# cjpurackal/nice-slam-cpp

Measured on AMD Instinct MI355X. Metric: mapping rays/sec (and ms/iter) on CoFusion room1 at 1/2/4/8 MI355X, higher is better.
Workload: dtype f32

## Files before the change

nice-slam-cpp_amd/csrc/nsk_train.h:

```cpp
#pragma once
#include "nsk_device.h"
#include <type_traits>
#include <utility>

#define PN_RB 272
#define PN_GROWS 32
#define PN_EROWS(CQ) (PN_GROWS + 16 * (CQ))
#define PN_ROWS(CQ) (PN_EROWS(CQ) + 96)
#define PN_MOFF(CQ) (PN_ROWS(CQ) * PN_RB)
#define PN_FLOATS(CQ) (2 * PN_MOFF(CQ) / 4)

struct TrainPhase {
    int RT, NC, rowsum;
    int slot0, nslots;
    int w_base, ld, col0;
    int rows, cols_total;
    int b_base;
};

template <int WHICH>
struct TrainPlan {
    static constexpr bool XYZ = WHICH != 0;
    static constexpr int CQ = WHICH == 2 ? 4 : 2;
    static constexpr int OD = WHICH == 3 ? 4 : 1;
// ... 191 lines not shown
                    else if (16 * ch + x < P.cols_total) g_dec[P.w_base + o * P.ld + P.col0 + 16 * ch + x] = v;
                }
            }
        }
    }
}

__device__ __forceinline__ void lds_barrier() { asm volatile("s_waitcnt lgkmcnt(0)\n\ts_barrier" ::: "memory"); }

template <int WHICH, bool RAYS, bool FULL = false>
__device__ __forceinline__ void decode_bwd_train_body(const DecArgs& A, int bid, int nb)
{
    constexpr bool XYZ = WHICH != 0;
    constexpr int CQ = WHICH == 2 ? 4 : 2;
    constexpr int OD = WHICH == 3 ? 4 : 1;
    constexpr bool SAVED = WHICH != 2;
    static_assert(FULL || WHICH == 0 || WHICH == 2, "the middle and colour decoders take this body only with FULL");
    typedef MlpFwdImg<CQ> FI;
    typedef TrainPlan<WHICH> PL;
    constexpr PL plan{};
    constexpr int BWD_F = XYZ ? MlpBwdImg::TOTAL : CoarseBwdImg::TOTAL;
    constexpr int IMG_F = SAVED ? BWD_F : 0;
    extern __shared__ __attribute__((aligned(16))) f4 smem[];
    const int wave = __builtin_amdgcn_readfirstlane(threadIdx.x >> 6), lane0 = threadIdx.x & 63;
    int lane = lane0, j = lane & 15, g = lane >> 4;
    float* smf = reinterpret_cast<float*>(smem);
    char* pn = reinterpret_cast<char*>(smf + IMG_F);
    constexpr int PM = PN_MOFF(CQ);
    float* scratch = smf + IMG_F + wave * 1056;
    copy_image_to_lds<512>(smem, A.bimg, IMG_F / 4);
    __syncthreads();
    const f4* fimg = A.img;
    const float* fimgf = reinterpret_cast<const float*>(fimg);
    const f4* bimg = SAVED ? smem : A.bimg;
    const float* bimgf = reinterpret_cast<const float*>(bimg);
    const float* Bm = nullptr;
    if constexpr (XYZ) Bm = SAVED ? bimgf + MlpBwdImg::P_BM : fimgf + FI::P_BM;
    const float* Bmb = Bm;
    const float* Wo = SAVED ? bimgf + (XYZ ? MlpBwdImg::P_WO : CoarseBwdImg::P_WO) : fimgf + FI::P_WO;

    f4 acc[plan.nslots];
#pragma unroll
    for (int k = 0; k < plan.nslots; ++k) acc[k] = (f4)(0.f);

    const int ntasks = (A.M + 15) >> 4;
    const int iters = tiles_per_wave(ntasks, nb * 8);
    const bool scat = (A.flags & 1u) && A.grid.g;
    struct Staged { float px, py, pz, zz; int n; bool valid; f4 gr; f4 xc[CQ]; f4 h4[2]; unsigned long long mask; } nx;
    auto task_of = [&](int it_) { return tile_of(it_, bid * 8 + wave, nb * 8); };
    auto slot_of = [&](int it_) { return task_of(it_) * 16 + j; };
    auto stage_a = [&](int it_, int mm, Staged& S_) {
        const int task = task_of(it_);
        const int slot = task * 16 + j;
        S_.valid = slot < A.M;
        sample_point(A, mm, S_.px, S_.py, S_.pz, S_.zz, S_.n);
        S_.gr = *reinterpret_cast<const f4*>(A.g_raw + (size_t)mm * 4);
        if constexpr (SAVED) {
            const int tk = min(task, ntasks - 1);
            S_.mask = A.masks[(size_t)min(slot, A.M - 1) * 4 + g];
            S_.h4[0] = A.hsave[((size_t)tk * 10 + 8) * 64 + lane]; S_.h4[1] = A.hsave[((size_t)tk * 10 + 9) * 64 + lane];
        }
    };
    auto stage_b = [&](Staged& S_) {
        Tri T_;
        tri_setup(A.grid, A.bound, S_.px, S_.py, S_.pz, T_);
        tri_gather(A.grid, T_, g, S_.xc[0], S_.xc[1]);
        if constexpr (WHICH == 2) {
            Tri Tm;
            tri_setup(A.grid_mid, A.bound, S_.px, S_.py, S_.pz, Tm);
            tri_gather(A.grid_mid, Tm, g, S_.xc[CQ - 2], S_.xc[CQ - 1]);
        }
    };
    int mm_next = 0;
    if (iters > 0) { stage_a(0, slot_sample(A, slot_of(0)), nx); stage_b(nx); mm_next = slot_sample(A, slot_of(1)); }
    if constexpr (SAVED) asm volatile("" : "+v"(nx.h4[0]), "+v"(nx.h4[1]), "+v"(nx.gr), "+v"(nx.mask), "+v"(mm_next));
    for (int it = 0; it < iters; ++it) {
        asm volatile("" ::: "memory");
        lane = lane0; asm volatile("" : "+v"(lane)); j = lane & 15; g = lane >> 4;
        if (it > 0) lds_barrier();
        const bool valid = nx.valid;
        float px = nx.px, py = nx.py, pz = nx.pz, zz = nx.zz; const int n = nx.n;
        Tri T;
        float gout[OD];
        {
            f4 gr = nx.gr;
            if (!valid) gr = (f4)(0.f);
            if constexpr (OD == 4) { gout[0] = gr[0]; gout[1] = gr[1]; gout[2] = gr[2]; gout[3] = 0.f; }
            else gout[0] = gr[3];
        }
        f4 go;
#pragma unroll
        for (int i = 0; i < 4; ++i) go[i] = (4 * g + i) < OD ? gout[(4 * g + i) < OD ? (4 * g + i) : 0] : 0.f;
        Act<CQ> C;
        ActC CC;
        f4 xcos[6];
        unsigned long long mask;
        const int htask = min(task_of(it), ntasks - 1);
        if constexpr (XYZ) {
#pragma unroll
            for (int q = 0; q < CQ; ++q) C.xc[q] = nx.xc[q];
            embed<false>(Bm, g, px, py, pz, C.xe, xcos);
#pragma unroll
            for (int q = 0; q < 6; ++q) pn_put(pn, PM, PN_EROWS(CQ) + 16 * q, wave, lane, C.xe[q]);
            if constexpr (SAVED) { C.h[4][0] = nx.h4[0]; C.h[4][1] = nx.h4[1]; mask = nx.mask; }
            else { mlp_forward<CQ>(fimg, lane, C); mask = C.mask; }
        } else {
            CC.xc[0] = nx.xc[0]; CC.xc[1] = nx.xc[1];
            CC.h[4][0] = nx.h4[0]; CC.h[4][1] = nx.h4[1]; mask = nx.mask;
        }
        f4 gh[2];
#pragma unroll
        for (int r = 0; r < 2; ++r)
#pragma unroll
            for (int i = 0; i < 4; ++i) {
                float s = 0.f;
#pragma unroll
                for (int o = 0; o < OD; ++o) s += Wo[32 * o + 16 * r + 4 * g + i] * gout[o];
                gh[r][i] = s;
            }
        {
            pn_put(pn, PM, 0, wave, lane, go);
            const f4* h4 = XYZ ? C.h[4] : CC.h[4];
            pn_put(pn, PM, PN_GROWS, wave, lane, h4[0]);
            pn_put(pn, PM, PN_GROWS + 16, wave, lane, h4[1]);
            lds_barrier();
            constexpr TrainPhase P = plan.p[PL::P_OUT];
            pn_tiles<P.nslots>(pn, PM, P.RT, P.NC, P.rowsum, wave, lane, acc + P.slot0);
            lds_barrier();
        }
        f4 gc[2] = {(f4)(0.f), (f4)(0.f)};
        f4 ge[6];
#pragma unroll
        for (int q = 0; q < 6; ++q) ge[q] = (f4)(0.f);
        auto load_h = [&](auto KC) {
            constexpr int k = decltype(KC)::value;
            const f4* src = A.hsave + ((size_t)htask * 10 + 2 * k) * 64 + lane;
            if constexpr (XYZ) { C.h[k][0] = src[0]; C.h[k][1] = src[64]; }
            else { CC.h[k][0] = src[0]; CC.h[k][1] = src[64]; }
        };
        if constexpr (SAVED) load_h(std::integral_constant<int, 3>{});
        auto layer = [&](auto LC) {
            constexpr int l = decltype(LC)::value;
            if constexpr (SAVED && l >= 2) load_h(std::integral_constant<int, l - 2>{});
            if constexpr (XYZ) {
                gemm<2, 2>(bimg, MlpBwdImg::FT(l), lane, gh, gc);
                pn_put(pn, PM, 0, wave, lane, gh[0]);
                pn_put(pn, PM, 16, wave, lane, gh[1]);
#pragma unroll
                for (int q = 0; q < CQ; ++q) pn_put(pn, PM, PN_GROWS + 16 * q, wave, lane, C.xc[q]);
                lds_barrier();
                constexpr TrainPhase P = plan.p[PL::P_FC0 + l];
                pn_tiles<P.nslots>(pn, PM, P.RT, P.NC, P.rowsum, wave, lane, acc + P.slot0);
                lds_barrier();
            }
            f4 ga[2];
#pragma unroll
            for (int r = 0; r < 2; ++r)
#pragma unroll
                for (int i = 0; i < 4; ++i) ga[r][i] = ((mask >> (8 * l + 4 * r + i)) & 1ull) ? gh[r][i] : 0.f;
            {
                pn_put(pn, PM, 0, wave, lane, ga[0]);
                pn_put(pn, PM, 16, wave, lane, ga[1]);
                if constexpr (XYZ) {
                    if constexpr (l == 0) {
                    } else if constexpr (l == 3) {
                        pn_put(pn, PM, PN_GROWS, wave, lane, C.h[2][0]);
                        pn_put(pn, PM, PN_GROWS + 16, wave, lane, C.h[2][1]);
                    } else {
                        pn_put(pn, PM, PN_GROWS, wave, lane, C.h[l - 1][0]);
                        pn_put(pn, PM, PN_GROWS + 16, wave, lane, C.h[l - 1][1]);
                    }
                } else {
                    if constexpr (l == 0 || l == 3) { pn_put(pn, PM, PN_GROWS, wave, lane, CC.xc[0]); pn_put(pn, PM, PN_GROWS + 16, wave, lane, CC.xc[1]); }
                    else { pn_put(pn, PM, PN_GROWS, wave, lane, CC.h[l - 1][0]); pn_put(pn, PM, PN_GROWS + 16, wave, lane, CC.h[l - 1][1]); }
                }
                lds_barrier();
                constexpr TrainPhase P = plan.p[PL::P_W0 + l];
                constexpr int xrow0 = (XYZ && (l == 0 || l == 3)) ? PN_EROWS(CQ) : PN_GROWS;
                pn_tiles<P.nslots>(pn, PM, P.RT, P.NC, P.rowsum, wave, lane, acc + P.slot0, xrow0);
                if constexpr (XYZ && l == 3) {
                    constexpr TrainPhase P2 = plan.p[PL::P_W3H];
                    pn_tiles<P2.nslots>(pn, PM, P2.RT, P2.NC, P2.rowsum, (wave + 4) & 7, lane, acc + P2.slot0);
                }
                lds_barrier();
                if constexpr (!XYZ && l == 3) {
                    const f4* h2 = CC.h[2];
                    pn_put(pn, PM, PN_GROWS, wave, lane, h2[0]);
                    pn_put(pn, PM, PN_GROWS + 16, wave, lane, h2[1]);
                    lds_barrier();
                    constexpr TrainPhase P2 = plan.p[PL::P_W3H];
                    pn_tiles<P2.nslots>(pn, PM, P2.RT, P2.NC, P2.rowsum, wave, lane, acc + P2.slot0);
                    lds_barrier();
                }
            }
            if constexpr (XYZ) {
                if constexpr (l == 3) gemm_e(bimg, MlpBwdImg::W3ET, lane, ga, ge);
                if constexpr (l == 0) gemm_e(bimg, MlpBwdImg::W0ET, lane, ga, ge);
                if constexpr (l >= 1) {
                    f4 ghn[2] = {(f4)(0.f), (f4)(0.f)};
                    gemm<2, 2>(bimg, MlpBwdImg::WT(l), lane, ga, ghn);
                    gh[0] = ghn[0]; gh[1] = ghn[1];
                }
            } else {
                if constexpr (l == 3) gemm<2, 2>(bimg, CoarseBwdImg::W3CT, lane, ga, gc);
                if constexpr (l == 0) gemm<2, 2>(bimg, CoarseBwdImg::W0T, lane, ga, gc);
                else {
                    constexpr int q0 = l == 1 ? CoarseBwdImg::W1T : (l == 2 ? CoarseBwdImg::W2T : (l == 3 ? CoarseBwdImg::W3HT : CoarseBwdImg::W4T));
                    f4 ghn[2] = {(f4)(0.f), (f4)(0.f)};
                    gemm<2, 2>(bimg, q0, lane, ga, ghn);
                    gh[0] = ghn[0]; gh[1] = ghn[1];
                }
            }
        };
        layer(std::integral_constant<int, 4>{});
        layer(std::integral_constant<int, 3>{});
        layer(std::integral_constant<int, 2>{});
        layer(std::integral_constant<int, 1>{});
        layer(std::integral_constant<int, 0>{});
        if (it + 1 < iters) { stage_a(it + 1, mm_next, nx); mm_next = slot_sample(A, slot_of(it + 2)); }
        float gp[3] = {0.f, 0.f, 0.f};
        asm volatile("" : "+v"(px), "+v"(py), "+v"(pz));
        tri_setup(A.grid, A.bound, px, py, pz, T);
        if constexpr (XYZ) {
            { f4 e2[6]; embed<true>(Bmb, g, px, py, pz, e2, xcos); }
#pragma unroll
            for (int q = 0; q < 6; ++q) ge[q] *= xcos[q];
            {
                f4 pq;
#pragma unroll
                for (int i = 0; i < 4; ++i) { int row = 4 * g + i; pq[i] = !valid ? 0.f : (row == 0 ? px : (row == 1 ? py : (row == 2 ? pz : 0.f))); }
                pn_put(pn, PM, 0, wave, lane, pq);
#pragma unroll
                for (int q = 0; q < 6; ++q) pn_put(pn, PM, PN_EROWS(CQ) + 16 * q, wave, lane, ge[q]);
                lds_barrier();
                constexpr TrainPhase P = plan.p[PL::P_DB];
                pn_tiles<P.nslots>(pn, PM, P.RT, P.NC, P.rowsum, wave, lane, acc + P.slot0, PN_EROWS(CQ));
                lds_barrier();
            }
            if constexpr (RAYS) {
#pragma unroll
                for (int q = 0; q < 6; ++q) {
                    f4 b0 = *reinterpret_cast<const f4*>(Bmb + 16 * q + 4 * g);
                    f4 b1 = *reinterpret_cast<const f4*>(Bmb + 96 + 16 * q + 4 * g);
                    f4 b2 = *reinterpret_cast<const f4*>(Bmb + 192 + 16 * q + 4 * g);
#pragma unroll
                    for (int i = 0; i < 4; ++i) { gp[0] += ge[q][i] * b0[i]; gp[1] += ge[q][i] * b1[i]; gp[2] += ge[q][i] * b2[i]; }
                }
            }
        }
        if constexpr (RAYS) {
            tri_grad_p(A.grid, T, g, gc, gp);
#pragma unroll
            for (int k = 0; k < 3; ++k) { gp[k] += __shfl_xor(gp[k], 16); gp[k] += __shfl_xor(gp[k], 32); }
            if (A.g_rays_o) {
                const int n0 = __builtin_amdgcn_readfirstlane(n);
                if (__builtin_amdgcn_ballot_w64(valid && n != n0) == 0ull) {
                    float a[6];
#pragma unroll
                    for (int k = 0; k < 3; ++k) { a[k] = valid ? gp[k] : 0.f; a[3 + k] = valid ? gp[k] * zz : 0.f; }
#pragma unroll
                    for (int o = 1; o < 16; o <<= 1)
#pragma unroll
                        for (int k = 0; k < 6; ++k) a[k] += __shfl_xor(a[k], o);
                    if (lane == 0) {
#pragma unroll
                        for (int k = 0; k < 3; ++k) { atomicAdd(A.g_rays_o + 3 * n0 + k, a[k]); atomicAdd(A.g_rays_d + 3 * n0 + k, a[3 + k]); }
                    }
                } else if (g == 0 && valid) {
#pragma unroll
                    for (int k = 0; k < 3; ++k) {
                        atomicAdd(A.g_rays_o + 3 * n + k, gp[k]);
                        atomicAdd(A.g_rays_d + 3 * n + k, gp[k] * zz);
                    }
                }
            }
        }
        if (it + 1 < iters) {
            stage_b(nx);
        }
        if constexpr (SAVED) asm volatile("" : "+v"(nx.h4[0]), "+v"(nx.h4[1]), "+v"(nx.gr), "+v"(nx.mask), "+v"(mm_next));
        if (scat) {
            if (A.flags & 0x8000u) {
                for (int w = 0; w < 8; ++w) { if (wave == w) { scatter_tile(A.grid, T, gc, lane, valid, scratch); asm volatile("s_waitcnt vmcnt(0)" ::: "memory"); } __syncthreads(); }
            } else scatter_tile(A.grid, T, gc, lane, valid, scratch);
        }
    }
    float* slab = A.g_dec + (size_t)bid * ((plan_total<WHICH>() + 3) & ~3);
    pn_flush<plan.p[PL::P_OUT].nslots>(slab, plan.p[PL::P_OUT], wave, lane, acc + plan.p[PL::P_OUT].slot0);
#define NSK_FLUSH(ID) if constexpr (plan.p[ID].nslots > 0) pn_flush<plan.p[ID].nslots>(slab, plan.p[ID], wave, lane, acc + plan.p[ID].slot0);
    NSK_FLUSH(1) NSK_FLUSH(2) NSK_FLUSH(3) NSK_FLUSH(4) NSK_FLUSH(5) NSK_FLUSH(6) NSK_FLUSH(7) NSK_FLUSH(8) NSK_FLUSH(9)
    NSK_FLUSH(10) NSK_FLUSH(12)
    if constexpr (plan.p[PL::P_W3H].nslots > 0)
        pn_flush<plan.p[PL::P_W3H].nslots>(slab, plan.p[PL::P_W3H], XYZ ? (wave + 4) & 7 : wave, lane, acc + plan.p[PL::P_W3H].slot0);
#undef NSK_FLUSH
}


#define PM_G1 0
#define PM_G2 32
#define PM_XC 64
#define PM_XH 96
#define PM_E 128
#define PM_ROWS 224
#define PM_IMG_FRAG_F (18 * 2 * 1024 / 4)
#define PM_IMG_F (PM_IMG_FRAG_F + 128 + 288)
#define PM_LDS_BYTES (PM_IMG_F * 4 + PM_ROWS * PN_RB * 2)

__device__ __forceinline__ void gemm_e2_lds(const h8* __restrict__ eimg, int lane, const H2& x3, const H2& x0, f4 (&acc)[6])
{
    constexpr int G3 = MlpBwdImgH::W3ET - MlpBwdImgH::W0ET;
#pragma unroll
    for (int a = 0; a < 3; ++a) {
        const FragH a30 = load_frag_h(eimg, G3 + 2 * a, lane), a31 = load_frag_h(eimg, G3 + 2 * a + 1, lane);
        const FragH a00 = load_frag_h(eimg, 2 * a, lane), a01 = load_frag_h(eimg, 2 * a + 1, lane);
        f4 tH[2] = {acc[2 * a], acc[2 * a + 1]}, tL[2] = {(f4)(0.f), (f4)(0.f)};
        mac_block_h(a30, a31, x3, tH, tL);
        mac_block_h(a00, a01, x0, tH, tL);
        acc[2 * a] = tH[0] + tL[0] * (1.f / NSK_H16_SCALE); acc[2 * a + 1] = tH[1] + tL[1] * (1.f / NSK_H16_SCALE);
    }
}
__device__ __forceinline__ void gemm_e2T_lds(const h8* __restrict__ eimg, int lane, const H2& x3, const H2& x0, f4 (&acc)[6])
{
    constexpr int G3 = MlpBwdImgH::W3ET - MlpBwdImgH::W0ET;
#pragma unroll
    for (int q = 0; q < 6; ++q) {
        const FragH f3 = load_frag_h(eimg, G3 + q, lane), f0 = load_frag_h(eimg, q, lane);
        f4 tH = (f4)(0.f), tL = (f4)(0.f);
        tH = mfma_h(x3.h, f3.h, tH); tL = mfma_h(x3.h, f3.l, tL); tL = mfma_h(x3.l, f3.h, tL);
        tH = mfma_h(x0.h, f0.h, tH); tL = mfma_h(x0.h, f0.l, tL); tL = mfma_h(x0.l, f0.h, tL);
        acc[q] = tH + tL * (1.f / NSK_H16_SCALE);
    }
}
typedef short s4v __attribute__((ext_vector_type(4)));
__device__ __forceinline__ f4 mfma_bf16_k16(unsigned a01, unsigned a23, unsigned b01, unsigned b23, f4 c)
{
    typedef unsigned int u2v __attribute__((ext_vector_type(2)));
    return __builtin_amdgcn_mfma_f32_16x16x16bf16_1k(__builtin_bit_cast(s4v, (u2v){a01, a23}), __builtin_bit_cast(s4v, (u2v){b01, b23}), c, 0, 0, 0);
}

struct TJob { int wave, grow, nt; int xrow[4]; int ph[4]; int rt; int ch[4]; };
template <int WHICH>
struct JobPlan {
    typedef TrainPlan<WHICH> PL;
    static constexpr int NJ = 32;
    static constexpr int PH_OUT = 0, PH_DB = 6;
    TJob j[NJ];
    int slot0[NJ];
    int first[8];
    int nslots;
    constexpr JobPlan() : j{}, slot0{}, first{}, nslots(0)
    {
        int n = 0;
        auto add = [&](int wave, int grow, int rt, int nt, int x0, int p0, int c0, int x1, int p1, int c1, int x2 = 0, int p2 = 0, int c2 = 0, int x3 = 0, int p3 = 0, int c3 = 0) {
            j[n] = TJob{wave, grow, nt, {x0, x1, x2, x3}, {p0, p1, p2, p3}, rt, {c0, c1, c2, c3}};
            ++n;
        };
        const int RS = -1;
        first[0] = n;
        add(0, PM_G1, 0, 3, PM_XH, PL::P_OUT, 0, PM_XH + 16, PL::P_OUT, 1, 0, PL::P_OUT, RS);
        for (int l = 4; l >= 0; --l) {
            first[1 + (4 - l)] = n;
            const int FC = PL::P_FC0 + l, W = PL::P_W0 + l;
            if (l == 4 || l == 2 || l == 1) {
                const int w0 = l == 4 ? 0 : 4;
                add(w0 + 0, PM_G1, 0, 3, PM_XC, FC, 0, PM_XC + 16, FC, 1, 0, FC, RS);
                add(w0 + 1, PM_G1 + 16, 1, 3, PM_XC, FC, 0, PM_XC + 16, FC, 1, 0, FC, RS);
                add(w0 + 2, PM_G2, 0, 3, PM_XH, W, 0, PM_XH + 16, W, 1, 0, W, RS);
                add(w0 + 3, PM_G2 + 16, 1, 3, PM_XH, W, 0, PM_XH + 16, W, 1, 0, W, RS);
            } else if (l == 3) {
                add(0, PM_G2, 0, 3, PM_E, W, 0, PM_E + 16, W, 1, 0, W, RS);
                add(4, PM_G1, 0, 3, PM_XC, FC, 0, PM_XC + 16, FC, 1, 0, FC, RS);
                add(1, PM_G2 + 16, 1, 3, PM_E, W, 0, PM_E + 16, W, 1, 0, W, RS);
                add(5, PM_G1 + 16, 1, 3, PM_XC, FC, 0, PM_XC + 16, FC, 1, 0, FC, RS);
                add(2, PM_G2, 0, 4, PM_E + 32, W, 2, PM_E + 48, W, 3, PM_XH, PL::P_W3H, 0, PM_XH + 16, PL::P_W3H, 1);
                add(6, PM_G2, 0, 2, PM_E + 64, W, 4, PM_E + 80, W, 5);
                add(3, PM_G2 + 16, 1, 4, PM_E + 32, W, 2, PM_E + 48, W, 3, PM_XH, PL::P_W3H, 0, PM_XH + 16, PL::P_W3H, 1);
                add(7, PM_G2 + 16, 1, 2, PM_E + 64, W, 4, PM_E + 80, W, 5);
            } else {
                add(0, PM_G2, 0, 3, PM_E, W, 0, PM_E + 16, W, 1, 0, W, RS);
                add(4, PM_G2, 0, 2, PM_E + 32, W, 2, PM_E + 48, W, 3);
                add(1, PM_G2 + 16, 1, 3, PM_E, W, 0, PM_E + 16, W, 1, 0, W, RS);
                add(5, PM_G2 + 16, 1, 2, PM_E + 32, W, 2, PM_E + 48, W, 3);
                add(2, PM_G1, 0, 3, PM_XC, FC, 0, PM_XC + 16, FC, 1, 0, FC, RS);
                add(6, PM_G2, 0, 2, PM_E + 64, W, 4, PM_E + 80, W, 5);
                add(3, PM_G1 + 16, 1, 3, PM_XC, FC, 0, PM_XC + 16, FC, 1, 0, FC, RS);
                add(7, PM_G2 + 16, 1, 2, PM_E + 64, W, 4, PM_E + 80, W, 5);
            }
        }
        first[6] = n;
        add(6, PM_G1, 0, 2, PM_E, PL::P_DB, 0, PM_E + 16, PL::P_DB, 1);
        add(7, PM_G1, 0, 2, PM_E + 32, PL::P_DB, 2, PM_E + 48, PL::P_DB, 3);
        add(1, PM_G1, 0, 2, PM_E + 64, PL::P_DB, 4, PM_E + 80, PL::P_DB, 5);
        first[7] = n;
        int used[8] = {0, 0, 0, 0, 0, 0, 0, 0};
        for (int q = 0; q < n; ++q) { slot0[q] = used[j[q].wave]; used[j[q].wave] += j[q].nt; }
        for (int w = 0; w < 8; ++w) nslots = used[w] > nslots ? used[w] : nslots;
    }
};

template <int WHICH>
constexpr bool jobplan_covers_plan()
{
    constexpr JobPlan<WHICH> JP{};
    constexpr TrainPlan<WHICH> plan{};
    for (int ph = 0; ph < TrainPlan<WHICH>::NPH; ++ph) {
        const TrainPhase P = plan.p[ph];
        for (int rt = 0; rt < P.RT; ++rt)
            for (int ch = -1; ch < P.NC; ++ch) {
                if (ch < 0 && !P.rowsum) continue;
                int owners = 0;
                for (int q = 0; q < JobPlan<WHICH>::NJ; ++q)
                    for (int k = 0; k < JP.j[q].nt; ++k)
                        if (JP.j[q].ph[k] == ph && JP.j[q].rt == rt && (ch < 0 ? JP.j[q].ch[k] < 0 : JP.j[q].ch[k] == ch)) ++owners;
                if (owners != 1) return false;
            }
    }
    int tiles = 0, want = 0;
    for (int q = 0; q < JobPlan<WHICH>::NJ; ++q) tiles += JP.j[q].nt;
    for (int ph = 0; ph < TrainPlan<WHICH>::NPH; ++ph) want += plan.p[ph].RT * plan.p[ph].NC + (plan.p[ph].rowsum ? plan.p[ph].RT : 0);
    return tiles == want && JP.nslots <= 12;
}
static_assert(jobplan_covers_plan<1>() && jobplan_covers_plan<3>(), "JobPlan: a weight-gradient tile is unowned, owned twice, or a wave holds more than 12 tiles");

template <int WHICH, int JJ>
__device__ __forceinline__ void pn_job(const char* __restrict__ pn, int moff, int wave, int lane, f4* acc)
{
    constexpr JobPlan<WHICH> JP{};
    constexpr TJob J = JP.j[JJ];
    constexpr int s0 = JP.slot0[JJ];
    if (wave != J.wave) return;
    const int r = lane & 15, sq = lane >> 4;
    const char* ga = pn + (J.grow + r) * PN_RB + 16 * sq;
    f4 d0[J.nt], d1[J.nt];
#pragma unroll
    for (int k = 0; k < J.nt; ++k) { d0[k] = acc[s0 + k]; d1[k] = (f4)(0.f); }
#pragma unroll
    for (int b = 0; b < 4; ++b) {
        const bf8 ah = *reinterpret_cast<const bf8*>(ga + 64 * b);
        const bf8 am = *reinterpret_cast<const bf8*>(ga + moff + 64 * b);
#pragma unroll
        for (int k = 0; k < J.nt; ++k) {
            if (J.ch[k] < 0) {
                const bf8 one = __builtin_bit_cast(bf8, (u4v)(0x3f803f80u));
                d0[k] = mfma_b(ah, one, d0[k]);
                d1[k] = mfma_b(am, one, d1[k]);
            } else {
                const char* xb = pn + (J.xrow[k] + r) * PN_RB + 16 * sq;
                const bf8 xh = *reinterpret_cast<const bf8*>(xb + 64 * b);
                const bf8 xm = *reinterpret_cast<const bf8*>(xb + moff + 64 * b);
                d0[k] = mfma_b(ah, xh, d0[k]);
                d1[k] = mfma_b(am, xm, d1[k]);
                d0[k] = mfma_b(ah, xm, d0[k]);
                d1[k] = mfma_b(am, xh, d1[k]);
            }
        }
    }
#pragma unroll
    for (int k = 0; k < J.nt; ++k) acc[s0 + k] = d0[k] + d1[k];
}
template <int WHICH, int J0, int... Is>
__device__ __forceinline__ void pn_jobs_seq(const char* __restrict__ pn, int moff, int wave, int lane, f4* acc, std::integer_sequence<int, Is...>)
{
    (pn_job<WHICH, J0 + Is>(pn, moff, wave, lane, acc), ...);
}
template <int WHICH, int PH>
__device__ __forceinline__ void pn_phase_jobs(const char* __restrict__ pn, int moff, int wave, int lane, f4* acc)
{
    constexpr JobPlan<WHICH> JP{};
    pn_jobs_seq<WHICH, JP.first[PH]>(pn, moff, wave, lane, acc, std::make_integer_sequence<int, JP.first[PH + 1] - JP.first[PH]>{});
}
template <int WHICH, int JJ, bool SKIP_DB>
__device__ __forceinline__ void pn_job_flush(float* __restrict__ g_dec, int wave, int lane, const f4* acc)
{
    constexpr JobPlan<WHICH> JP{};
    constexpr TrainPlan<WHICH> plan{};
    constexpr TJob J = JP.j[JJ];
    constexpr int s0 = JP.slot0[JJ];
    if (wave != J.wave) return;
    const int x = lane & 15, g = lane >> 4;
#pragma unroll
    for (int k = 0; k < J.nt; ++k) {
        const TrainPhase P = plan.p[J.ph[k]];
        if (SKIP_DB && J.ph[k] == TrainPlan<WHICH>::P_DB) continue;
        const bool rs = J.ch[k] < 0;
#pragma unroll
        for (int i = 0; i < 4; ++i) {
            const int o = 16 * J.rt + 4 * g + i;
            const float v = acc[s0 + k][i];
            if (o < P.rows) {
                if (rs) { if (x == 0) g_dec[P.b_base + o] = v; }
                else if (16 * J.ch[k] + x < P.cols_total) g_dec[P.w_base + o * P.ld + P.col0 + 16 * J.ch[k] + x] = v;
            }
        }
    }
}
template <int WHICH, bool SKIP_DB, int... Is>
__device__ __forceinline__ void pn_jobs_flush_all(float* __restrict__ g_dec, int wave, int lane, const f4* acc, std::integer_sequence<int, Is...>)
{
    (pn_job_flush<WHICH, Is, SKIP_DB>(g_dec, wave, lane, acc), ...);
}

template <int WHICH, bool RAYS>
__device__ __forceinline__ void decode_bwd_train_m_body(const DecArgs& A, int bid, int nb)
{
    static_assert(WHICH == 1 || WHICH == 3, "merged-phase body: middle and colour decoders");
    constexpr int CQ = 2;
    constexpr int OD = WHICH == 3 ? 4 : 1;
    typedef TrainPlan<WHICH> PL;
    constexpr PL plan{};
    extern __shared__ __attribute__((aligned(16))) f4 smem[];
    const int wave = __builtin_amdgcn_readfirstlane(threadIdx.x >> 6), lane0 = threadIdx.x & 63;
    int lane = lane0, j = lane & 15, g = lane >> 4;
    float* smf = reinterpret_cast<float*>(smem);
    char* pn = reinterpret_cast<char*>(smf + PM_IMG_F);
    constexpr int PM = PM_ROWS * PN_RB;
    float* scratch = smf + PM_IMG_F + wave * 1056;
    static_assert(8 * 1056 * 4 <= PM_E * PN_RB, "scatter scratch must end before the E rows");
    const h8* imgh = reinterpret_cast<const h8*>(smem);
    const f4* gimg_e = reinterpret_cast<const f4*>(A.bimg16) + (size_t)MlpBwdImgH::W0ET * 2 * 1024 / 16;
    constexpr int EIMG_F4 = 12 * 2 * 1024 / 16;
    static_assert(EIMG_F4 == 3 * 512 && EIMG_F4 * 16 <= (PM_E - PM_G2) * PN_RB, "e-part image: three float4 per thread, inside plane H of rows 32..127");
    f4* eimg = reinterpret_cast<f4*>(pn + PM_G2 * PN_RB);
    const h8* eimgh = reinterpret_cast<const h8*>(eimg);
    const float* Wo = smf + PM_IMG_FRAG_F;
    const float* Bm = Wo + 128;

    constexpr JobPlan<WHICH> JP{};
    f4 acc[JP.nslots];
#pragma unroll
    for (int k = 0; k < JP.nslots; ++k) acc[k] = (f4)(0.f);

    const int ntasks = (A.M + 15) >> 4;
    const int iters = tiles_per_wave(ntasks, nb * 8);
    const bool scat = (A.flags & 1u) && A.grid.g;
    struct Staged { SampleRaw r; float px, py, pz; int mm; bool valid; f4 gr; f4 xc[CQ]; f4 h4[2]; unsigned long long mask; } nx;
    auto task_of = [&](int it_) { return tile_of(it_, bid * 8 + wave, nb * 8); };
    auto slot_of = [&](int it_) { return task_of(it_) * 16 + j; };
    auto stage_a = [&](int it_, int mm, Staged& S_) {
        const int task = task_of(it_);
        const int slot = task * 16 + j;
        S_.valid = slot < A.M;
        S_.mm = mm;
        sample_load(A, mm, S_.r);
        S_.gr = ld32<f4>(A.g_raw, (unsigned)mm * 16u);
        const int tk = min(task, ntasks - 1);
        S_.mask = ld32<unsigned long long>(A.masks, ((unsigned)min(slot, A.M - 1) * 4u + (unsigned)g) * 8u);
        S_.h4[0] = A.hsave[((size_t)tk * 10 + 8) * 64 + lane]; S_.h4[1] = A.hsave[((size_t)tk * 10 + 9) * 64 + lane];
    };
    Tri Tn; GatherRaw GR;
    auto stage_b1 = [&](Staged& S_) {
        sample_finish(A, S_.r, S_.px, S_.py, S_.pz);
        tri_setup(A.grid, A.bound, S_.px, S_.py, S_.pz, Tn);
        tri_gather_issue(A.grid, Tn, g, GR);
    };
    auto stage_b2 = [&](Staged& S_) { tri_gather_reduce(Tn, GR, S_.xc[0], S_.xc[1]); };
    int mm_next = 0;
    {
        const f4* src = reinterpret_cast<const f4*>(A.bimg16);
        constexpr int K0 = (PM_IMG_FRAG_F / 4 + 511) / 512;
        ImgRegs<K0> ir0; ImgRegs<1> ir1;
        const int mm0 = slot_sample(A, slot_of(0));
        image_issue<512>(ir0, src, PM_IMG_FRAG_F / 4);
        image_issue<512>(ir1, src + MlpBwdImgH::P_WO / 4, (128 + 288) / 4);
        if (iters > 0) stage_a(0, mm0, nx);
        image_commit<512>(smem, ir0, src, PM_IMG_FRAG_F / 4);
        image_commit<512>(smem + PM_IMG_FRAG_F / 4, ir1, src + MlpBwdImgH::P_WO / 4, (128 + 288) / 4);
        __syncthreads();
        if (iters > 0) { stage_b1(nx); stage_b2(nx); mm_next = slot_sample(A, slot_of(1)); }
    }
    asm volatile("" : "+v"(nx.h4[0]), "+v"(nx.h4[1]), "+v"(nx.gr), "+v"(nx.mask), "+v"(mm_next));
    f4 accB[2] = {(f4)(0.f), (f4)(0.f)};
    (void)accB;
    for (int it = 0; it < iters; ++it) {
        asm volatile("" ::: "memory");
        lane = lane0; asm volatile("" : "+v"(lane)); j = lane & 15; g = lane >> 4;
        if (it > 0) lds_barrier();
        const bool valid = nx.valid;
        float px = nx.px, py = nx.py, pz = nx.pz, zz = A.pts ? 0.f : nx.r.z; const int n = A.pts ? 0 : ray_of(A, nx.mm);
        (void)zz; (void)n;
        float gout[OD];
        {
            f4 gr = nx.gr;
            if (!valid) gr = (f4)(0.f);
            if constexpr (OD == 4) { gout[0] = gr[0]; gout[1] = gr[1]; gout[2] = gr[2]; gout[3] = 0.f; }
            else gout[0] = gr[3];
        }
        f4 go;
#pragma unroll
        for (int i = 0; i < 4; ++i) go[i] = (4 * g + i) < OD ? gout[(4 * g + i) < OD ? (4 * g + i) : 0] : 0.f;
        const float us = chain_scale<OD>(gout);
        const unsigned long long mask = nx.mask;
        const int htask = min(task_of(it), ntasks - 1);
        f4 hq[5][2];
        hq[4][0] = nx.h4[0]; hq[4][1] = nx.h4[1];
        auto load_h = [&](auto KC) {
            constexpr int k = decltype(KC)::value;
            const f4* src = A.hsave + ((size_t)htask * 10 + 2 * k) * 64 + lane;
            hq[k][0] = src[0]; hq[k][1] = src[64];
        };
        load_h(std::integral_constant<int, 3>{});
        {
            f4 xe[6], dummy[6];
            embed<false>(Bm, g, px, py, pz, xe, dummy);
#pragma unroll
            for (int q = 0; q < 6; ++q) pn_put(pn, PM, PM_E + 16 * q, wave, lane, xe[q]);
        }
        pn_put(pn, PM, PM_XC, wave, lane, nx.xc[0]);
        pn_put(pn, PM, PM_XC + 16, wave, lane, nx.xc[1]);
        f4 gh[2];
#pragma unroll
        for (int r = 0; r < 2; ++r)
#pragma unroll
            for (int i = 0; i < 4; ++i) {
                float s = 0.f;
#pragma unroll
                for (int o = 0; o < OD; ++o) s += Wo[32 * o + 16 * r + 4 * g + i] * gout[o];
                gh[r][i] = s;
            }
        {
            pn_put(pn, PM, PM_G1, wave, lane, go);
            pn_put(pn, PM, PM_XH, wave, lane, hq[4][0]);
            pn_put(pn, PM, PM_XH + 16, wave, lane, hq[4][1]);
            lds_barrier();
            pn_phase_jobs<WHICH, JobPlan<WHICH>::PH_OUT>(pn, PM, wave, lane, acc);
            lds_barrier();
        }
        f4 gc[2] = {(f4)(0.f), (f4)(0.f)};
        H2 xa3, xa;
        auto layer = [&](auto LC) {
            constexpr int l = decltype(LC)::value;
            if constexpr (l >= 2) load_h(std::integral_constant<int, l - 2>{});
            const Mask4 RM = relu_mask_dwords(mask, l);
            {
                const H2 xg = split_block_h(gh[0], gh[1]);
                f4 gl[2] = {(f4)(0.f), (f4)(0.f)};
                gemm_h(imgh, MlpBwdImgH::FT(l), lane, xg, gc, gl);
                gc[0] += gl[0] * (1.f / NSK_H16_SCALE); gc[1] += gl[1] * (1.f / NSK_H16_SCALE);
                xa = mask_block_h4(xg, RM);
            }
            pn_put_masked(pn, PM, PM_G1, PM_G2, wave, lane, gh[0], us, RM.d[0], RM.d[1]);
            pn_put_masked(pn, PM, PM_G1 + 16, PM_G2 + 16, wave, lane, gh[1], us, RM.d[2], RM.d[3]);
            if constexpr (l >= 1) {
                constexpr int k = l == 3 ? 2 : l - 1;
                pn_put(pn, PM, PM_XH, wave, lane, hq[k][0]);
                pn_put(pn, PM, PM_XH + 16, wave, lane, hq[k][1]);
            }
            lds_barrier();
            pn_phase_jobs<WHICH, 1 + (4 - l)>(pn, PM, wave, lane, acc);
            lds_barrier();
            if constexpr (l == 3) xa3 = xa;
            if constexpr (l >= 1) {
                f4 ghn[2] = {(f4)(0.f), (f4)(0.f)}, ghl[2] = {(f4)(0.f), (f4)(0.f)};
                gemm_h(imgh, MlpBwdImgH::WT(l), lane, xa, ghn, ghl);
                gh[0] = ghn[0] + ghl[0] * (1.f / NSK_H16_SCALE); gh[1] = ghn[1] + ghl[1] * (1.f / NSK_H16_SCALE);
            }
        };
        layer(std::integral_constant<int, 4>{});
        layer(std::integral_constant<int, 3>{});
        layer(std::integral_constant<int, 2>{});
        layer(std::integral_constant<int, 1>{});
        f4 ecp[3];
#pragma unroll
        for (int u = 0; u < 3; ++u) ecp[u] = gimg_e[u * 512 + (int)threadIdx.x];
        layer(std::integral_constant<int, 0>{});
#pragma unroll
        for (int u = 0; u < 3; ++u) eimg[u * 512 + (int)threadIdx.x] = ecp[u];
        lds_barrier();
        gc[0] *= us; gc[1] *= us;
        float gp[3] = {0.f, 0.f, 0.f};
        Tri T;
        f4 ge[6];
        if constexpr (!RAYS) {
            if (it + 1 < iters) { stage_a(it + 1, mm_next, nx); mm_next = slot_sample(A, slot_of(it + 2)); }
            gemm_e2T_lds(eimgh, lane, xa3, xa, ge);
            stage_b1(nx);
            float* xch = reinterpret_cast<float*>(pn + PM + PM_G1 * PN_RB) + wave * 64;
            if (g == 0) *reinterpret_cast<f4*>(xch + 4 * j) = (f4){px, py, pz, valid ? us : 0.f};
            asm volatile("s_waitcnt lgkmcnt(0)" ::: "memory");
            const int nb3 = j / 3, nc = j - 3 * nb3;
            unsigned ph01, pm01, ph23, pm23;
            f4 sp[4];
#pragma unroll
            for (int i = 0; i < 4; ++i) sp[i] = *reinterpret_cast<const f4*>(xch + 4 * (4 * g + i));
            {
                float pv[4];
#pragma unroll
                for (int i = 0; i < 4; ++i) pv[i] = (nc == 0 ? sp[i][0] : (nc == 1 ? sp[i][1] : sp[i][2])) * sp[i][3];
                split2_pair(pv[0], pv[1], ph01, pm01); split2_pair(pv[2], pv[3], ph23, pm23);
            }
#pragma unroll
            for (int q = 0; q < 6; ++q) {
                const int f = 16 * q + j;
                const float b0 = Bm[f], b1 = Bm[96 + f], b2 = Bm[192 + f];
                float gs[4];
#pragma unroll
                for (int i = 0; i < 4; ++i) {
                    const float s = add_rn(add_rn(mul_rn(sp[i][0], b0), mul_rn(sp[i][1], b1)), mul_rn(sp[i][2], b2));
                    const float cv = __builtin_amdgcn_cosf(nsk_rev(s));
                    gs[i] = f < NSK_E ? ge[q][i] * cv : 0.f;
                }
                unsigned ah01, am01, ah23, am23;
                split2_pair(gs[0], gs[1], ah01, am01); split2_pair(gs[2], gs[3], ah23, am23);
                const bool on = nb3 == (q % 5);
                const unsigned bh01 = on ? ph01 : 0u, bh23 = on ? ph23 : 0u, bm01 = on ? pm01 : 0u, bm23 = on ? pm23 : 0u;
                f4& d = accB[q / 5];
                d = mfma_bf16_k16(ah01, ah23, bh01, bh23, d);
                d = mfma_bf16_k16(ah01, ah23, bm01, bm23, d);
                d = mfma_bf16_k16(am01, am23, bh01, bh23, d);
                d = mfma_bf16_k16(am01, am23, bm01, bm23, d);
            }
            tri_setup(A.grid, A.bound, px, py, pz, T);
        } else {
#pragma unroll
            for (int q = 0; q < 6; ++q) ge[q] = (f4)(0.f);
            gemm_e2_lds(eimgh, lane, xa3, xa, ge);
            if (it + 1 < iters) { stage_a(it + 1, mm_next, nx); mm_next = slot_sample(A, slot_of(it + 2)); }
            tri_setup(A.grid, A.bound, px, py, pz, T);
            {
                f4 e2[6], xcos[6];
                embed<true>(Bm, g, px, py, pz, e2, xcos);
#pragma unroll
                for (int q = 0; q < 6; ++q) ge[q] *= xcos[q];
            }
            {
                f4 pq;
#pragma unroll
                for (int i = 0; i < 4; ++i) { int row = 4 * g + i; pq[i] = !valid ? 0.f : (row == 0 ? px : (row == 1 ? py : (row == 2 ? pz : 0.f))); }
                pn_put(pn, PM, PM_G1, wave, lane, pq, us);
#pragma unroll
                for (int q = 0; q < 6; ++q) pn_put(pn, PM, PM_E + 16 * q, wave, lane, ge[q]);
                stage_b1(nx);
                lds_barrier();
                pn_phase_jobs<WHICH, JobPlan<WHICH>::PH_DB>(pn, PM, wave, lane, acc);
                lds_barrier();
            }
        }
        if constexpr (RAYS) {
#pragma unroll
            for (int q = 0; q < 6; ++q) {
                f4 b0 = *reinterpret_cast<const f4*>(Bm + 16 * q + 4 * g);
                f4 b1 = *reinterpret_cast<const f4*>(Bm + 96 + 16 * q + 4 * g);
                f4 b2 = *reinterpret_cast<const f4*>(Bm + 192 + 16 * q + 4 * g);
#pragma unroll
                for (int i = 0; i < 4; ++i) { gp[0] += ge[q][i] * b0[i]; gp[1] += ge[q][i] * b1[i]; gp[2] += ge[q][i] * b2[i]; }
            }
            gp[0] *= us; gp[1] *= us; gp[2] *= us;
            tri_grad_p(A.grid, T, g, gc, gp);
#pragma unroll
            for (int k = 0; k < 3; ++k) { gp[k] += __shfl_xor(gp[k], 16); gp[k] += __shfl_xor(gp[k], 32); }
            if (A.g_rays_o) {
                const int n0 = __builtin_amdgcn_readfirstlane(n);
                if (__builtin_amdgcn_ballot_w64(valid && n != n0) == 0ull) {
                    float a[6];
#pragma unroll
                    for (int k = 0; k < 3; ++k) { a[k] = valid ? gp[k] : 0.f; a[3 + k] = valid ? gp[k] * zz : 0.f; }
#pragma unroll
                    for (int o = 1; o < 16; o <<= 1)
#pragma unroll
                        for (int k = 0; k < 6; ++k) a[k] += __shfl_xor(a[k], o);
                    if (lane == 0) {
#pragma unroll
                        for (int k = 0; k < 3; ++k) { atomicAdd(A.g_rays_o + 3 * n0 + k, a[k]); atomicAdd(A.g_rays_d + 3 * n0 + k, a[3 + k]); }
                    }
                } else if (g == 0 && valid) {
#pragma unroll
                    for (int k = 0; k < 3; ++k) {
                        atomicAdd(A.g_rays_o + 3 * n + k, gp[k]);
                        atomicAdd(A.g_rays_d + 3 * n + k, gp[k] * zz);
                    }
                }
            }
        }
        stage_b2(nx);
        asm volatile("" : "+v"(nx.h4[0]), "+v"(nx.h4[1]), "+v"(nx.gr), "+v"(nx.mask), "+v"(mm_next), "+v"(nx.xc[0]), "+v"(nx.xc[1]));
        if (scat) {
            if (A.flags & 0x8000u) {
                for (int w = 0; w < 8; ++w) { if (wave == w) { scatter_tile(A.grid, T, gc, lane, valid, scratch); asm volatile("s_waitcnt vmcnt(0)" ::: "memory"); } __syncthreads(); }
            } else scatter_tile(A.grid, T, gc, lane, valid, scratch);
        }
    }
    float* slab = A.g_dec + (size_t)bid * ((plan_total<WHICH>() + 3) & ~3);
    pn_jobs_flush_all<WHICH, !RAYS>(slab, wave, lane, acc, std::make_integer_sequence<int, JobPlan<WHICH>::NJ>{});
    if constexpr (!RAYS) {
        __syncthreads();
        f4* red = reinterpret_cast<f4*>(pn);
        red[(wave * 2 + 0) * 64 + lane] = accB[0]; red[(wave * 2 + 1) * 64 + lane] = accB[1];
        __syncthreads();
        if (threadIdx.x < 128) {
            const int a = threadIdx.x >> 6;
            f4 v = red[a * 64 + lane];
#pragma unroll
            for (int w = 1; w < 8; ++w) v += red[(w * 2 + a) * 64 + lane];
            constexpr TrainPhase P = plan.p[PL::P_DB];
            const int q = a == 0 ? j / 3 : 5, k = j - 3 * (j / 3);
            if (a == 0 ? j < 15 : j < 3) {
#pragma unroll
                for (int i = 0; i < 4; ++i) {
                    const int f = 16 * q + 4 * g + i;
                    if (f < NSK_E) slab[P.w_base + k * P.ld + f] = v[i];
                }
            }
        }
    }
}

template <int WHICH, bool RAYS>
__device__ __forceinline__ void decode_bwd_train_any(const DecArgs& A, int bid, int nb)
{
    if constexpr (WHICH == 1 || WHICH == 3) decode_bwd_train_m_body<WHICH, RAYS>(A, bid, nb);
    else decode_bwd_train_body<WHICH, RAYS>(A, bid, nb);
}

template <int WHICH, bool RAYS>
__global__ __launch_bounds__(512) void k_decode_bwd_train(DecArgs A) { decode_bwd_train_any<WHICH, RAYS>(A, blockIdx.x, gridDim.x); }

template <bool RAYS>
__global__ __launch_bounds__(512) void k_decode_bwd_multi(MultiArgs MA)
{
    if (MA.sum_n > 0 && blockIdx.x == gridDim.x - 1) { block_sum(MA.sum_src, MA.sum_n, MA.sum_dst); return; }
    if constexpr (!RAYS) {
        if ((int)blockIdx.x >= MA.wg_end[MA.n - 1]) { sort_scan_body<2>(MA.scan, (int)blockIdx.x - MA.wg_end[MA.n - 1]); return; }
    }
    int r = 0;
    while (r < MA.n - 1 && (int)blockIdx.x >= MA.wg_end[r]) ++r;
    const int b0 = r == 0 ? 0 : MA.wg_end[r - 1];
    const int bid = blockIdx.x - b0, nb = MA.wg_end[r] - b0;
    const int sel = MA.which[r] * 2 + (MA.train[r] ? 1 : 0);
    switch (sel) {
    case 0: decode_bwd_body<0, RAYS>(MA.a[r], bid, nb); break;
    case 1: decode_bwd_train_any<0, RAYS>(MA.a[r], bid, nb); break;
    case 2: if constexpr (RAYS) decode_bwd_body<1, RAYS>(MA.a[r], bid, nb); else decode_bwd_frozen_role<1, 8>(MA, r, bid, nb); break;
    case 3: decode_bwd_train_any<1, RAYS>(MA.a[r], bid, nb); break;
    case 4: if constexpr (RAYS) decode_bwd_body<2, RAYS>(MA.a[r], bid, nb); else decode_bwd_frozen_role<2, 8>(MA, r, bid, nb); break;
    case 5: break;
    case 6: if constexpr (RAYS) decode_bwd_body<3, RAYS>(MA.a[r], bid, nb); else decode_bwd_frozen_role<3, 8>(MA, r, bid, nb); break;
    default: decode_bwd_train_any<3, RAYS>(MA.a[r], bid, nb); break;
    }
}

template <bool RAYS>
__global__ __launch_bounds__(512) void k_decode_bwd_multi_full(MultiArgs MA)
{
    if (MA.sum_n > 0 && blockIdx.x == gridDim.x - 1) { block_sum(MA.sum_src, MA.sum_n, MA.sum_dst); return; }
    int r = 0;
    while (r < MA.n - 1 && (int)blockIdx.x >= MA.wg_end[r]) ++r;
    const int b0 = r == 0 ? 0 : MA.wg_end[r - 1];
    const int bid = blockIdx.x - b0, nb = MA.wg_end[r] - b0;
    const int sel = MA.which[r] * 2 + (MA.train[r] ? 1 : 0);
    switch (sel) {
    case 0: decode_bwd_body<0, RAYS, 8, true>(MA.a[r], bid, nb); break;
    case 1: decode_bwd_train_body<0, RAYS, true>(MA.a[r], bid, nb); break;
    case 2: decode_bwd_body<1, RAYS, 8, true>(MA.a[r], bid, nb); break;
    case 3: decode_bwd_train_body<1, RAYS, true>(MA.a[r], bid, nb); break;
    case 4: decode_bwd_body<2, RAYS, 8, true>(MA.a[r], bid, nb); break;
    case 5: break;
    case 6: decode_bwd_body<3, RAYS, 8, true>(MA.a[r], bid, nb); break;
    default: decode_bwd_train_body<3, RAYS, true>(MA.a[r], bid, nb); break;
    }
}
```

Baseline: 14.60 million.

## Merge output-layer weight-gradient phase into layer-0 phase via dedicated GO rows

```diff
diff --git a/nice-slam-cpp_amd/csrc/nsk_train.h b/nice-slam-cpp_amd/csrc/nsk_train.h
--- a/nice-slam-cpp_amd/csrc/nsk_train.h
+++ b/nice-slam-cpp_amd/csrc/nsk_train.h
@@ -517,9 +517,12 @@
 #define PM_XH 96
 #define PM_E 128
 #define PM_ROWS 224
+#define PM_GO (2 * PM_ROWS)
+#define PM_GO_ROWS 4
 #define PM_IMG_FRAG_F (18 * 2 * 1024 / 4)
 #define PM_IMG_F (PM_IMG_FRAG_F + 128 + 288)
-#define PM_LDS_BYTES (PM_IMG_F * 4 + PM_ROWS * PN_RB * 2)
+#define PM_LDS_BYTES (PM_IMG_F * 4 + PM_ROWS * PN_RB * 2 + PM_GO_ROWS * PN_RB * 2)
+static_assert(PM_LDS_BYTES <= 160 * 1024 - 256, "merged-phase body: image + panel + GO must fit the CU's 160 KiB less the scan rider's static words (k_decode_bwd_multi<false>)");
 
 __device__ __forceinline__ void gemm_e2_lds(const h8* __restrict__ eimg, int lane, const H2& x3, const H2& x0, f4 (&acc)[6])
 {
@@ -557,11 +560,11 @@
 template <int WHICH>
 struct JobPlan {
     typedef TrainPlan<WHICH> PL;
-    static constexpr int NJ = 32;
-    static constexpr int PH_OUT = 0, PH_DB = 6;
+    static constexpr int NJ = 31;
+    static constexpr int PH_DB = 5;
     TJob j[NJ];
     int slot0[NJ];
-    int first[8];
+    int first[7];
     int nslots;
     constexpr JobPlan() : j{}, slot0{}, first{}, nslots(0)
     {
@@ -571,10 +574,8 @@
             ++n;
         };
         const int RS = -1;
-        first[0] = n;
-        add(0, PM_G1, 0, 3, PM_XH, PL::P_OUT, 0, PM_XH + 16, PL::P_OUT, 1, 0, PL::P_OUT, RS);
         for (int l = 4; l >= 0; --l) {
-            first[1 + (4 - l)] = n;
+            first[4 - l] = n;
             const int FC = PL::P_FC0 + l, W = PL::P_W0 + l;
             if (l == 4 || l == 2 || l == 1) {
                 const int w0 = l == 4 ? 0 : 4;
@@ -592,21 +593,21 @@
                 add(3, PM_G2 + 16, 1, 4, PM_E + 32, W, 2, PM_E + 48, W, 3, PM_XH, PL::P_W3H, 0, PM_XH + 16, PL::P_W3H, 1);
                 add(7, PM_G2 + 16, 1, 2, PM_E + 64, W, 4, PM_E + 80, W, 5);
             } else {
-                add(0, PM_G2, 0, 3, PM_E, W, 0, PM_E + 16, W, 1, 0, W, RS);
-                add(4, PM_G2, 0, 2, PM_E + 32, W, 2, PM_E + 48, W, 3);
+                add(0, PM_GO, 0, 3, PM_XH, PL::P_OUT, 0, PM_XH + 16, PL::P_OUT, 1, 0, PL::P_OUT, RS);
+                add(4, PM_G2, 0, 3, PM_E, W, 0, PM_E + 16, W, 1, 0, W, RS);
                 add(1, PM_G2 + 16, 1, 3, PM_E, W, 0, PM_E + 16, W, 1, 0, W, RS);
-                add(5, PM_G2 + 16, 1, 2, PM_E + 32, W, 2, PM_E + 48, W, 3);
-                add(2, PM_G1, 0, 3, PM_XC, FC, 0, PM_XC + 16, FC, 1, 0, FC, RS);
-                add(6, PM_G2, 0, 2, PM_E + 64, W, 4, PM_E + 80, W, 5);
+                add(5, PM_G1, 0, 3, PM_XC, FC, 0, PM_XC + 16, FC, 1, 0, FC, RS);
+                add(2, PM_G2 + 16, 1, 4, PM_E + 32, W, 2, PM_E + 48, W, 3, PM_E + 64, W, 4, PM_E + 80, W, 5);
+                add(6, PM_G2, 0, 2, PM_E + 32, W, 2, PM_E + 48, W, 3);
                 add(3, PM_G1 + 16, 1, 3, PM_XC, FC, 0, PM_XC + 16, FC, 1, 0, FC, RS);
-                add(7, PM_G2 + 16, 1, 2, PM_E + 64, W, 4, PM_E + 80, W, 5);
-            }
-        }
-        first[6] = n;
+                add(7, PM_G2, 0, 2, PM_E + 64, W, 4, PM_E + 80, W, 5);
+            }
+        }
+        first[5] = n;
         add(6, PM_G1, 0, 2, PM_E, PL::P_DB, 0, PM_E + 16, PL::P_DB, 1);
         add(7, PM_G1, 0, 2, PM_E + 32, PL::P_DB, 2, PM_E + 48, PL::P_DB, 3);
         add(1, PM_G1, 0, 2, PM_E + 64, PL::P_DB, 4, PM_E + 80, PL::P_DB, 5);
-        first[7] = n;
+        first[6] = n;
         int used[8] = {0, 0, 0, 0, 0, 0, 0, 0};
         for (int q = 0; q < n; ++q) { slot0[q] = used[j[q].wave]; used[j[q].wave] += j[q].nt; }
         for (int w = 0; w < 8; ++w) nslots = used[w] > nslots ? used[w] : nslots;
@@ -636,6 +637,16 @@
     return tiles == want && JP.nslots <= 12;
 }
 static_assert(jobplan_covers_plan<1>() && jobplan_covers_plan<3>(), "JobPlan: a weight-gradient tile is unowned, owned twice, or a wave holds more than 12 tiles");
+template <int WHICH>
+constexpr bool jobplan_layer0_dealt()
+{
+    constexpr JobPlan<WHICH> JP{};
+    int simd[4] = {0, 0, 0, 0}, tiles = 0;
+    for (int q = JP.first[4]; q < JP.first[5]; ++q) { simd[JP.j[q].wave & 3] += JP.j[q].nt; tiles += JP.j[q].nt; }
+    for (int s = 0; s < 4; ++s) if (simd[s] > 6) return false;
+    return tiles == 23;
+}
+static_assert(jobplan_layer0_dealt<1>() && jobplan_layer0_dealt<3>(), "JobPlan: layer 0's phase must carry 23 tiles, no SIMD more than six");
 
 template <int WHICH, int JJ>
 __device__ __forceinline__ void pn_job(const char* __restrict__ pn, int moff, int wave, int lane, f4* acc)
@@ -645,14 +656,21 @@
     constexpr int s0 = JP.slot0[JJ];
     if (wave != J.wave) return;
     const int r = lane & 15, sq = lane >> 4;
-    const char* ga = pn + (J.grow + r) * PN_RB + 16 * sq;
+    constexpr bool GO = J.grow == PM_GO;
+    const bool live = !GO || r < PM_GO_ROWS;
+    const char* ga = pn + (J.grow + (live ? r : 0)) * PN_RB + 16 * sq;
+    const int gmoff = GO ? PM_GO_ROWS * PN_RB : moff;
     f4 d0[J.nt], d1[J.nt];
 #pragma unroll
     for (int k = 0; k < J.nt; ++k) { d0[k] = acc[s0 + k]; d1[k] = (f4)(0.f); }
 #pragma unroll
     for (int b = 0; b < 4; ++b) {
-        const bf8 ah = *reinterpret_cast<const bf8*>(ga + 64 * b);
-        const bf8 am = *reinterpret_cast<const bf8*>(ga + moff + 64 * b);
+        bf8 ah = *reinterpret_cast<const bf8*>(ga + 64 * b);
+        bf8 am = *reinterpret_cast<const bf8*>(ga + gmoff + 64 * b);
+        if constexpr (GO) {
+            const u4v z = (u4v)(0u);
+            ah = live ? ah : __builtin_bit_cast(bf8, z); am = live ? am : __builtin_bit_cast(bf8, z);
+        }
 #pragma unroll
         for (int k = 0; k < J.nt; ++k) {
             if (J.ch[k] < 0) {
@@ -678,6 +696,20 @@
 {
     (pn_job<WHICH, J0 + Is>(pn, moff, wave, lane, acc), ...);
 }
+__device__ __forceinline__ void pn_put_go(char* __restrict__ pn, int wave, int lane, f4 x)
+{
+    const PairSel P = pair_sel(wave, lane);
+    char* ph = pn + (PM_GO + (P.odd ? 2 : 0)) * PN_RB + P.col2;
+    unsigned h01, m01, h23, m23, ha, hb, ma, mb;
+    split2_pair(x[0], x[1], h01, m01);
+    split2_pair(x[2], x[3], h23, m23);
+    pair_words(h01, h23, P.odd, P.selA, P.selB, ha, hb);
+    pair_words(m01, m23, P.odd, P.selA, P.selB, ma, mb);
+    if (lane < 16) {
+        *reinterpret_cast<unsigned*>(ph) = ha; *reinterpret_cast<unsigned*>(ph + PN_RB) = hb;
+        *reinterpret_cast<unsigned*>(ph + PM_GO_ROWS * PN_RB) = ma; *reinterpret_cast<unsigned*>(ph + (PM_GO_ROWS + 1) * PN_RB) = mb;
+    }
+}
 template <int WHICH, int PH>
 __device__ __forceinline__ void pn_phase_jobs(const char* __restrict__ pn, int moff, int wave, int lane, f4* acc)
 {
@@ -731,6 +763,9 @@
     constexpr int PM = PM_ROWS * PN_RB;
     float* scratch = smf + PM_IMG_F + wave * 1056;
     static_assert(8 * 1056 * 4 <= PM_E * PN_RB, "scatter scratch must end before the E rows");
+    static_assert(PM_GO * PN_RB >= 2 * PM && PM_IMG_F * 4 + (PM_GO + 2 * PM_GO_ROWS) * PN_RB == PM_LDS_BYTES,
+                  "GO: behind both planes of the panel (so clear of the scatter scratch, the e-part image copy and the xch rows, which the asserts here keep inside a plane), inside the allocation");
+    static_assert(PM_G1 * PN_RB + 8 * 64 * 4 <= PM, "xch exchange rows: inside plane M");
     const h8* imgh = reinterpret_cast<const h8*>(smem);
     const f4* gimg_e = reinterpret_cast<const f4*>(A.bimg16) + (size_t)MlpBwdImgH::W0ET * 2 * 1024 / 16;
     constexpr int EIMG_F4 = 12 * 2 * 1024 / 16;
@@ -748,7 +783,7 @@
     const int ntasks = (A.M + 15) >> 4;
     const int iters = tiles_per_wave(ntasks, nb * 8);
     const bool scat = (A.flags & 1u) && A.grid.g;
-    struct Staged { SampleRaw r; float px, py, pz; int mm; bool valid; f4 gr; f4 xc[CQ]; f4 h4[2]; unsigned long long mask; } nx;
+    struct Staged { SampleRaw r; float px, py, pz; int mm; bool valid; f4 gr; f4 xc[CQ]; unsigned long long mask; } nx;
     auto task_of = [&](int it_) { return tile_of(it_, bid * 8 + wave, nb * 8); };
     auto slot_of = [&](int it_) { return task_of(it_) * 16 + j; };
     auto stage_a = [&](int it_, int mm, Staged& S_) {
@@ -758,9 +793,7 @@
         S_.mm = mm;
         sample_load(A, mm, S_.r);
         S_.gr = ld32<f4>(A.g_raw, (unsigned)mm * 16u);
-        const int tk = min(task, ntasks - 1);
         S_.mask = ld32<unsigned long long>(A.masks, ((unsigned)min(slot, A.M - 1) * 4u + (unsigned)g) * 8u);
-        S_.h4[0] = A.hsave[((size_t)tk * 10 + 8) * 64 + lane]; S_.h4[1] = A.hsave[((size_t)tk * 10 + 9) * 64 + lane];
     };
     Tri Tn; GatherRaw GR;
     auto stage_b1 = [&](Staged& S_) {
@@ -783,7 +816,7 @@
         __syncthreads();
         if (iters > 0) { stage_b1(nx); stage_b2(nx); mm_next = slot_sample(A, slot_of(1)); }
     }
-    asm volatile("" : "+v"(nx.h4[0]), "+v"(nx.h4[1]), "+v"(nx.gr), "+v"(nx.mask), "+v"(mm_next));
+    asm volatile("" : "+v"(nx.gr), "+v"(nx.mask), "+v"(mm_next));
     f4 accB[2] = {(f4)(0.f), (f4)(0.f)};
     (void)accB;
     for (int it = 0; it < iters; ++it) {
@@ -807,7 +840,6 @@
         const unsigned long long mask = nx.mask;
         const int htask = min(task_of(it), ntasks - 1);
         f4 hq[5][2];
-        hq[4][0] = nx.h4[0]; hq[4][1] = nx.h4[1];
         auto load_h = [&](auto KC) {
             constexpr int k = decltype(KC)::value;
             const f4* src = A.hsave + ((size_t)htask * 10 + 2 * k) * 64 + lane;
@@ -832,19 +864,13 @@
                 for (int o = 0; o < OD; ++o) s += Wo[32 * o + 16 * r + 4 * g + i] * gout[o];
                 gh[r][i] = s;
             }
-        {
-            pn_put(pn, PM, PM_G1, wave, lane, go);
-            pn_put(pn, PM, PM_XH, wave, lane, hq[4][0]);
-            pn_put(pn, PM, PM_XH + 16, wave, lane, hq[4][1]);
-            lds_barrier();
-            pn_phase_jobs<WHICH, JobPlan<WHICH>::PH_OUT>(pn, PM, wave, lane, acc);
-            lds_barrier();
-        }
+        pn_put_go(pn, wave, lane, go);
         f4 gc[2] = {(f4)(0.f), (f4)(0.f)};
         H2 xa3, xa;
         auto layer = [&](auto LC) {
             constexpr int l = decltype(LC)::value;
             if constexpr (l >= 2) load_h(std::integral_constant<int, l - 2>{});
+            if constexpr (l == 1) load_h(std::integral_constant<int, 4>{});
             const Mask4 RM = relu_mask_dwords(mask, l);
             {
                 const H2 xg = split_block_h(gh[0], gh[1]);
@@ -855,13 +881,13 @@
             }
             pn_put_masked(pn, PM, PM_G1, PM_G2, wave, lane, gh[0], us, RM.d[0], RM.d[1]);
             pn_put_masked(pn, PM, PM_G1 + 16, PM_G2 + 16, wave, lane, gh[1], us, RM.d[2], RM.d[3]);
-            if constexpr (l >= 1) {
-                constexpr int k = l == 3 ? 2 : l - 1;
+            {
+                constexpr int k = l == 3 ? 2 : (l == 0 ? 4 : l - 1);
                 pn_put(pn, PM, PM_XH, wave, lane, hq[k][0]);
                 pn_put(pn, PM, PM_XH + 16, wave, lane, hq[k][1]);
             }
             lds_barrier();
-            pn_phase_jobs<WHICH, 1 + (4 - l)>(pn, PM, wave, lane, acc);
+            pn_phase_jobs<WHICH, 4 - l>(pn, PM, wave, lane, acc);
             lds_barrier();
             if constexpr (l == 3) xa3 = xa;
             if constexpr (l >= 1) {
@@ -987,7 +1013,7 @@
             }
         }
         stage_b2(nx);
-        asm volatile("" : "+v"(nx.h4[0]), "+v"(nx.h4[1]), "+v"(nx.gr), "+v"(nx.mask), "+v"(mm_next), "+v"(nx.xc[0]), "+v"(nx.xc[1]));
+        asm volatile("" : "+v"(nx.gr), "+v"(nx.mask), "+v"(mm_next), "+v"(nx.xc[0]), "+v"(nx.xc[1]));
         if (scat) {
             if (A.flags & 0x8000u) {
                 for (int w = 0; w < 8; ++w) { if (wave == w) { scatter_tile(A.grid, T, gc, lane, valid, scratch); asm volatile("s_waitcnt vmcnt(0)" ::: "memory"); } __syncthreads(); }
```

Result: no change. 14.66 million (median of 6 runs) (+0.4%).
